# yanivw12/gs2mesh

Hardware: AMD Instinct MI355X
Metric: stereo-pair renders/sec + TSDF Mvoxel-updates/sec (higher is better)
Workload: dtype f32

## Files before the change

### gs2mesh_amd/csrc/tsdf_api.hip

```cpp
#include <math.h>
#include <stdio.h>
#include <string.h>

#include <mutex>
#include <vector>

#include "../../include/gs2mesh_amd.h"
#include "tsdf_common.h"
#include "tsdf_internal.h"
#include "roctx_ranges.h"

#define HIPCHK(expr)                                                                          \
    do {                                                                                      \
        hipError_t e__ = (expr);                                                              \
        if (e__ != hipSuccess) {                                                              \
            gs2m_set_error("%s failed: %s (%s:%d)", #expr, hipGetErrorString(e__), __FILE__, __LINE__); \
            return 1;                                                                         \
        }                                                                                     \
    } while (0)

struct gs2m_tsdf {
    int device = 0;
    double voxel_length = 0, sdf_trunc = 0, unit_length = 0;
    int color_type = 1, resolution = 16, stride = 4;
// ... 30 lines not shown

static hipEvent_t tsdf_ev_get(gs2m_tsdf* t) {
    if (!t->ev_free.empty()) {
        hipEvent_t e = t->ev_free.back();
        t->ev_free.pop_back();
        return e;
    }
    hipEvent_t e;
    if (hipEventCreate(&e) != hipSuccess) return nullptr;
    return e;
}

static bool invert4x4(const double* m, double* inv) {
    double a[16];
    a[0] = m[5] * m[10] * m[15] - m[5] * m[11] * m[14] - m[9] * m[6] * m[15] + m[9] * m[7] * m[14] + m[13] * m[6] * m[11] - m[13] * m[7] * m[10];
    a[4] = -m[4] * m[10] * m[15] + m[4] * m[11] * m[14] + m[8] * m[6] * m[15] - m[8] * m[7] * m[14] - m[12] * m[6] * m[11] + m[12] * m[7] * m[10];
    a[8] = m[4] * m[9] * m[15] - m[4] * m[11] * m[13] - m[8] * m[5] * m[15] + m[8] * m[7] * m[13] + m[12] * m[5] * m[11] - m[12] * m[7] * m[9];
    a[12] = -m[4] * m[9] * m[14] + m[4] * m[10] * m[13] + m[8] * m[5] * m[14] - m[8] * m[6] * m[13] - m[12] * m[5] * m[10] + m[12] * m[6] * m[9];
    a[1] = -m[1] * m[10] * m[15] + m[1] * m[11] * m[14] + m[9] * m[2] * m[15] - m[9] * m[3] * m[14] - m[13] * m[2] * m[11] + m[13] * m[3] * m[10];
    a[5] = m[0] * m[10] * m[15] - m[0] * m[11] * m[14] - m[8] * m[2] * m[15] + m[8] * m[3] * m[14] + m[12] * m[2] * m[11] - m[12] * m[3] * m[10];
    a[9] = -m[0] * m[9] * m[15] + m[0] * m[11] * m[13] + m[8] * m[1] * m[15] - m[8] * m[3] * m[13] - m[12] * m[1] * m[11] + m[12] * m[3] * m[9];
    a[13] = m[0] * m[9] * m[14] - m[0] * m[10] * m[13] - m[8] * m[1] * m[14] + m[8] * m[2] * m[13] + m[12] * m[1] * m[10] - m[12] * m[2] * m[9];
    a[2] = m[1] * m[6] * m[15] - m[1] * m[7] * m[14] - m[5] * m[2] * m[15] + m[5] * m[3] * m[14] + m[13] * m[2] * m[7] - m[13] * m[3] * m[6];
    a[6] = -m[0] * m[6] * m[15] + m[0] * m[7] * m[14] + m[4] * m[2] * m[15] - m[4] * m[3] * m[14] - m[12] * m[2] * m[7] + m[12] * m[3] * m[6];
    a[10] = m[0] * m[5] * m[15] - m[0] * m[7] * m[13] - m[4] * m[1] * m[15] + m[4] * m[3] * m[13] + m[12] * m[1] * m[7] - m[12] * m[3] * m[5];
    a[14] = -m[0] * m[5] * m[14] + m[0] * m[6] * m[13] + m[4] * m[1] * m[14] - m[4] * m[2] * m[13] - m[12] * m[1] * m[6] + m[12] * m[2] * m[5];
    a[3] = -m[1] * m[6] * m[11] + m[1] * m[7] * m[10] + m[5] * m[2] * m[11] - m[5] * m[3] * m[10] - m[9] * m[2] * m[7] + m[9] * m[3] * m[6];
    a[7] = m[0] * m[6] * m[11] - m[0] * m[7] * m[10] - m[4] * m[2] * m[11] + m[4] * m[3] * m[10] + m[8] * m[2] * m[7] - m[8] * m[3] * m[6];
    a[11] = -m[0] * m[5] * m[11] + m[0] * m[7] * m[9] + m[4] * m[1] * m[11] - m[4] * m[3] * m[9] - m[8] * m[1] * m[7] + m[8] * m[3] * m[5];
    a[15] = m[0] * m[5] * m[10] - m[0] * m[6] * m[9] - m[4] * m[1] * m[10] + m[4] * m[2] * m[9] + m[8] * m[1] * m[6] - m[8] * m[2] * m[5];
    double det = m[0] * a[0] + m[1] * a[4] + m[2] * a[8] + m[3] * a[12];
    if (det == 0) return false;
    det = 1.0 / det;
    for (int i = 0; i < 16; i++) inv[i] = a[i] * det;
    return true;
}

static int zero_state(gs2m_tsdf* t, hipStream_t st, bool whole_pool, long long keep_first = -1) {
    TsdfVolume& V = t->V;
    if (whole_pool) {
        HIPCHK(hipMemsetAsync(V.tsdf, 0, sizeof(float) * (size_t)V.max_blocks * GS2M_TSDF_VOX, st));
        HIPCHK(hipMemsetAsync(V.weight, 0, sizeof(float) * (size_t)V.max_blocks * GS2M_TSDF_VOX, st));
        if (V.rgb) HIPCHK(hipMemsetAsync(V.rgb, 0, sizeof(unsigned) * 3 * (size_t)V.max_blocks * GS2M_TSDF_VOX, st));
        HIPCHK(hipMemsetAsync(V.halo, 0, (size_t)V.max_blocks, st));
    } else if (keep_first < 0) {
        gs2m_launch_tsdf_clear_used(st, V);
    } else {
        gs2m_launch_tsdf_clear_from(st, V, (unsigned)keep_first);
    }
    HIPCHK(hipMemsetAsync(V.hash_keys, 0xff, sizeof(unsigned long long) * (size_t)V.hash_cap, st));
    HIPCHK(hipMemsetAsync(V.hash_vals, 0xff, sizeof(int) * (size_t)V.hash_cap, st));
    HIPCHK(hipMemsetAsync(V.stamp, 0, sizeof(unsigned) * (size_t)V.hash_cap, st));
    HIPCHK(hipMemsetAsync(V.fmask, 0, sizeof(unsigned long long) * (size_t)V.hash_cap, st));
    HIPCHK(hipMemsetAsync(V.counters, 0, sizeof(unsigned) * 4, st));
    HIPCHK(hipMemsetAsync(V.totals, 0, sizeof(unsigned long long), st));
    return 0;
}

extern "C" int gs2m_tsdf_create(gs2m_tsdf** out, double voxel_length, double sdf_trunc, int color_type,
                                int volume_unit_resolution, int depth_sampling_stride, int64_t max_blocks,
                                int device) {
    if (!out) {
        gs2m_set_error("gs2m_tsdf_create: out is NULL");
        return 1;
    }
    if (volume_unit_resolution != GS2M_TSDF_RES) {
        gs2m_set_error("volume_unit_resolution %d not supported (kernels are specialised for 16, Open3D's default)",
                       volume_unit_resolution);
        return 1;
    }
    if (!(voxel_length > 0) || !(sdf_trunc > 0) || depth_sampling_stride < 1 || max_blocks < 1 ||
        max_blocks > (1ll << 30) || (color_type != GS2M_TSDF_COLOR_NONE && color_type != GS2M_TSDF_COLOR_RGB8)) {
        gs2m_set_error("gs2m_tsdf_create: bad argument");
        return 1;
    }
    HIPCHK(hipSetDevice(device));
    gs2m_tsdf* t = new gs2m_tsdf();
    t->device = device;
    t->voxel_length = voxel_length;
    t->sdf_trunc = sdf_trunc;
    t->unit_length = voxel_length * volume_unit_resolution;
    t->color_type = color_type;
    t->stride = depth_sampling_stride;
    memset(&t->V, 0, sizeof(t->V));
    TsdfVolume& V = t->V;
    V.max_blocks = (unsigned)max_blocks;
    unsigned cap = 1024;
    while ((uint64_t)cap < 2ull * (uint64_t)max_blocks) cap <<= 1;
    V.hash_cap = cap;
    V.has_color = color_type == GS2M_TSDF_COLOR_RGB8;
    const size_t nvox = (size_t)max_blocks * GS2M_TSDF_VOX;
    bool ok = hipMalloc((void**)&V.tsdf, sizeof(float) * nvox) == hipSuccess &&
              hipMalloc((void**)&V.weight, sizeof(float) * nvox) == hipSuccess &&
              (!V.has_color || hipMalloc((void**)&V.rgb, sizeof(unsigned) * 3 * nvox) == hipSuccess) &&
              hipMalloc((void**)&V.block_keys, sizeof(int) * 3 * (size_t)max_blocks) == hipSuccess &&
              hipMalloc((void**)&V.halo, (size_t)max_blocks) == hipSuccess &&
              hipMalloc((void**)&V.hash_keys, sizeof(unsigned long long) * (size_t)cap) == hipSuccess &&
              hipMalloc((void**)&V.hash_vals, sizeof(int) * (size_t)cap) == hipSuccess &&
              hipMalloc((void**)&V.stamp, sizeof(unsigned) * (size_t)cap) == hipSuccess &&
              hipMalloc((void**)&V.touched, sizeof(unsigned) * (size_t)cap) == hipSuccess &&
              hipMalloc((void**)&V.fmask, sizeof(unsigned long long) * (size_t)cap) == hipSuccess &&
              hipMalloc((void**)&t->d_bframes, sizeof(TsdfBatchFrame) * GS2M_TSDF_MAX_BATCH) == hipSuccess &&
              hipHostMalloc((void**)&t->h_bframes, sizeof(TsdfBatchFrame) * GS2M_TSDF_MAX_BATCH * gs2m_tsdf::kRing) == hipSuccess &&
              hipMalloc((void**)&V.counters, sizeof(unsigned) * 4) == hipSuccess &&
              hipMalloc((void**)&V.totals, sizeof(unsigned long long)) == hipSuccess &&
              hipMalloc((void**)&t->d_mc, gs2m_mc_tables_bytes()) == hipSuccess &&
              hipMalloc((void**)&t->d_blk_tris, sizeof(unsigned) * (size_t)max_blocks) == hipSuccess &&
              hipMalloc((void**)&t->d_ntri, sizeof(unsigned long long)) == hipSuccess &&
              hipHostMalloc((void**)&t->h_counters, sizeof(unsigned) * 4) == hipSuccess &&
              hipHostMalloc((void**)&t->h_totals, sizeof(unsigned long long)) == hipSuccess;
    if (!ok) {
        gs2m_set_error("gs2m_tsdf_create: out of device memory for %lld blocks (%.1f MiB)", (long long)max_blocks,
                       (double)nvox * 20.0 / 1048576.0);
        gs2m_tsdf_destroy(t);
        return 1;
    }
    {
        std::vector<unsigned char> tab(gs2m_mc_tables_bytes());
        if (!gs2m_mc_tables_fill(tab.data()) ||
            hipMemcpy(t->d_mc, tab.data(), tab.size(), hipMemcpyHostToDevice) != hipSuccess) {
            gs2m_set_error("gs2m_tsdf_create: marching-cubes table generation failed");
            gs2m_tsdf_destroy(t);
            return 1;
        }
    }
    if (zero_state(t, (hipStream_t)0, true)) {
        gs2m_tsdf_destroy(t);
        return 1;
    }
    HIPCHK(hipStreamSynchronize((hipStream_t)0));
    *out = t;
    return 0;
}

extern "C" int gs2m_tsdf_destroy(gs2m_tsdf* t) {
    if (!t) return 0;
    TsdfVolume& V = t->V;
    (void)hipFree(V.tsdf);
    (void)hipFree(V.weight);
    (void)hipFree(V.rgb);
    (void)hipFree(V.block_keys);
    (void)hipFree(V.halo);
    (void)hipFree(V.hash_keys);
    (void)hipFree(V.hash_vals);
    (void)hipFree(V.stamp);
    (void)hipFree(V.touched);
    (void)hipFree(V.fmask);
    (void)hipFree(t->d_bframes);
    (void)hipHostFree(t->h_bframes);
    for (auto e : t->ring_done)
        if (e) (void)hipEventDestroy(e);
    (void)hipFree(V.counters);
    (void)hipFree(V.totals);
    (void)hipFree(t->d_mc);
    (void)hipFree(t->d_blk_tris);
    (void)hipFree(t->d_ntri);
    (void)hipFree(t->mesh_scratch);
// ... 111 lines not shown
    }
    {
        Gs2mRange rg("gs2m:tsdf_integrate");
        gs2m_launch_tsdf_integrate(st, t->n_cu * 7, t->V, f, depth, color, mask);
    }
    if (tm) {
        (void)hipEventRecord(e3, st);
        t->ev_live.push_back({0, e0, e1, 1});
        t->ev_live.push_back({1, e2, e3, 1});
    }
    return 0;
}

extern "C" int gs2m_tsdf_integrate_batch(gs2m_tsdf* t, int n_frames, const float* const* depth, const uint8_t* const* color,
                                         const uint8_t* const* mask, int width, int height, double fx, double fy, double cx,
                                         double cy, const double* extrinsics_w2c, double depth_scale, double depth_trunc,
                                         double min_depth, gs2m_stream stream) {
    if (!t || n_frames < 0 || (n_frames > 0 && (!depth || !extrinsics_w2c))) {
        gs2m_set_error("gs2m_tsdf_integrate_batch: NULL argument");
        return 1;
    }
    if (t->V.has_color && n_frames > 0 && !color) {
        gs2m_set_error("[ScalableTSDFVolume::Integrate] Unsupported image format.");
        return 1;
    }
    if (n_frames > 0 && (width <= 0 || height <= 0 || width > 65535 || height > 65535 || !(fx != 0) || !(fy != 0) || !(depth_scale != 0))) {
        gs2m_set_error("gs2m_tsdf_integrate_batch: bad intrinsics / size (the sweep packs pixel coordinates in 16 bits: <= 65535)");
        return 1;
    }
    HIPCHK(hipSetDevice(t->device));
    hipStream_t st = (hipStream_t)stream;
    for (int f0 = 0; f0 < n_frames; f0 += GS2M_TSDF_MAX_BATCH) {
        const int nf = n_frames - f0 < GS2M_TSDF_MAX_BATCH ? n_frames - f0 : GS2M_TSDF_MAX_BATCH;
        const unsigned slot = t->ring_next++ % gs2m_tsdf::kRing;
        if (t->ring_done[slot]) HIPCHK(hipEventSynchronize(t->ring_done[slot]));
        else HIPCHK(hipEventCreateWithFlags(&t->ring_done[slot], hipEventDisableTiming));
        TsdfBatchFrame* hb = t->h_bframes + (size_t)slot * GS2M_TSDF_MAX_BATCH;
        for (int k = 0; k < nf; ++k) {
            const int i = f0 + k;
            if (!depth[i] || (t->V.has_color && !color[i])) {
                gs2m_set_error("gs2m_tsdf_integrate_batch: frame %d has a NULL image", i);
                return 1;
            }
            const unsigned char* m = mask ? mask[i] : nullptr;
            if (fill_frame(t, hb[k].f, width, height, fx, fy, cx, cy, extrinsics_w2c + 16 * (size_t)i, depth_scale, depth_trunc,
                           min_depth, m != nullptr))
                return 1;
            hb[k].depth = depth[i];
            hb[k].color = color ? color[i] : nullptr;
            hb[k].mask = m;
        }
        HIPCHK(hipMemcpyAsync(t->d_bframes, hb, sizeof(TsdfBatchFrame) * nf, hipMemcpyHostToDevice, st));
        HIPCHK(hipEventRecord(t->ring_done[slot], st));
        HIPCHK(hipMemsetAsync(t->V.counters + 1, 0, sizeof(unsigned), st));
        HIPCHK(hipMemsetAsync(t->V.counters + 3, 0, sizeof(unsigned), st));
        hipEvent_t e0 = nullptr, e1 = nullptr, e2 = nullptr, e3 = nullptr;
        if (t->timing) {
            e0 = tsdf_ev_get(t);
            e1 = tsdf_ev_get(t);
            e2 = tsdf_ev_get(t);
            e3 = tsdf_ev_get(t);
        }
        const bool tm = e0 && e1 && e2 && e3;
        if (tm) (void)hipEventRecord(e0, st);
        {
            Gs2mRange rg("gs2m:tsdf_touch_batch");
            gs2m_launch_tsdf_touch_batch(st, t->V, hb[0].f, nf, t->d_bframes);
        }
        if (tm) {
            (void)hipEventRecord(e1, st);
            (void)hipEventRecord(e2, st);
        }
        {
            Gs2mRange rg("gs2m:tsdf_integrate_batch");
            gs2m_launch_tsdf_integrate_batch(st, t->n_cu, t->V, t->d_bframes);
        }
        if (tm) {
            (void)hipEventRecord(e3, st);
            t->ev_live.push_back({0, e0, e1, nf});
            t->ev_live.push_back({1, e2, e3, nf});
        }
    }
    return 0;
}

extern "C" int gs2m_tsdf_set_stage_timing(gs2m_tsdf* t, int enable) {
    if (!t) {
        gs2m_set_error("null handle");
        return 1;
    }
    t->timing = enable != 0;
    return 0;
}

extern "C" int gs2m_tsdf_stage_times(gs2m_tsdf* t, gs2m_stream stream, double* total_ms, int64_t* launches) {
    if (!t || !total_ms || !launches) {
        gs2m_set_error("gs2m_tsdf_stage_times: NULL argument");
        return 1;
    }
    HIPCHK(hipStreamSynchronize((hipStream_t)stream));
    for (auto& p : t->ev_live) {
        float ms = 0.f;
        if (hipEventElapsedTime(&ms, p.a, p.b) == hipSuccess && (p.stage == 0 || p.stage == 1)) {
            total_ms[p.stage] += ms;
            launches[p.stage] += p.frames;
        }
        t->ev_free.push_back(p.a);
        t->ev_free.push_back(p.b);
// ... 504 lines not shown
```

### gs2mesh_amd/csrc/tsdf_common.h

```cpp
#pragma once
#include "platform.h"

#define GS2M_TSDF_RES 16
#define GS2M_TSDF_VOX 4096
#define GS2M_TSDF_EMPTY 0xffffffffffffffffull
#define GS2M_TSDF_KEY_BIAS (1 << 20)

struct TsdfVolume {
    float* tsdf;
    float* weight;
    unsigned* rgb;
    int* block_keys;
    unsigned char* halo;
    unsigned long long* hash_keys;
    int* hash_vals;
    unsigned* stamp;
    unsigned* touched;
    unsigned long long* fmask;
    unsigned* counters;
    unsigned long long* totals;
    unsigned hash_cap;
    unsigned max_blocks;
    int has_color;
};

struct TsdfFrame {
    double pose[12];
    double fx, fy, cx, cy;
    double unit_length, sdf_trunc, depth_trunc;
    float E[12];
    float fx_f, fy_f, cx_f, cy_f, fx_inv_f, fy_inv_f;
    float voxel_length_f, half_voxel_length_f, sdf_trunc_f, sdf_trunc_inv_f;
    float Es02, Es12, Es22;
    float safe_w, safe_h;
    float depth_scale_f, min_depth_f;
    float depth_trunc_up_f;
    int W, H, stride, nx, ny;
    unsigned frame_id;
    int use_mask, use_min;
};

struct TsdfBatchFrame {
    TsdfFrame f;
    const float* depth;
    const unsigned char* color;
    const unsigned char* mask;
};
#define GS2M_TSDF_MAX_BATCH 64

#define GS2M_TSDF_VINDEX(x, y, z) (((((z) >> 2) * 16 + ((x) >> 2) * 4 + ((y) >> 2)) * 64) + ((z)&3) * 16 + ((x)&3) * 4 + ((y)&3))

GS2M_DEVICE unsigned long long tsdf_pack_key(int bx, int by, int bz) {
    return ((unsigned long long)(unsigned)(bx + GS2M_TSDF_KEY_BIAS) << 42) |
           ((unsigned long long)(unsigned)(by + GS2M_TSDF_KEY_BIAS) << 21) |
           (unsigned long long)(unsigned)(bz + GS2M_TSDF_KEY_BIAS);
}
GS2M_DEVICE bool tsdf_key_in_range(int bx, int by, int bz) {
    const int B = GS2M_TSDF_KEY_BIAS;
    return bx >= -B && bx < B && by >= -B && by < B && bz >= -B && bz < B;
}
GS2M_DEVICE unsigned tsdf_hash(unsigned long long k) {
    k ^= k >> 33;
    k *= 0xff51afd7ed558ccdull;
    k ^= k >> 33;
    k *= 0xc4ceb9fe1a85ec53ull;
    k ^= k >> 33;
    return (unsigned)k;
}
```

### gs2mesh_amd/csrc/tsdf_kernels.h

```cpp
#pragma once
#include "tsdf_common.h"

GS2M_DEVICE float tsdf_fetch_depth(const float* __restrict__ depth, const unsigned char* __restrict__ mask,
                                   const TsdfFrame& f, int u, int v) {
    const size_t p = (size_t)v * f.W + u;
    float d = depth[p];
    if (f.use_mask && mask[p] == 0) d = d * 0.0f;
    if (f.use_min && d < f.min_depth_f) d = 0.0f;
    if (f.depth_scale_f != 1.0f) d /= f.depth_scale_f;
    if (d >= f.depth_trunc_up_f) d = 0.0f;
    return d;
}

GS2M_DEVICE unsigned tsdf_find_or_insert(const TsdfVolume& V, unsigned long long key, int bx, int by, int bz) {
    const unsigned mask = V.hash_cap - 1u;
    unsigned h = tsdf_hash(key) & mask;
    for (unsigned probe = 0; probe < V.hash_cap; ++probe, h = (h + 1u) & mask) {
        unsigned long long k = V.hash_keys[h];
        if (k == key) return h;
        if (k == GS2M_TSDF_EMPTY) {
            const unsigned long long prev = atomicCAS(&V.hash_keys[h], GS2M_TSDF_EMPTY, key);
            if (prev == GS2M_TSDF_EMPTY) {
                const unsigned slot = atomicAdd(&V.counters[0], 1u);
                if (slot < V.max_blocks) {
// ... 103 lines not shown
        return;
    }
    const int ny = whi[1] - wlo[1] + 1, nz = whi[2] - wlo[2] + 1;
    const int nyz = ny * nz;
    const int total = (int)total_ll;
    for (int base = 0; base < total; base += 64) {
        const int c = base + lane;
        if (c >= total) continue;
        const int cx = c / nyz, rem = c - cx * nyz;
        const int cy = rem / nz;
        const int bx = wlo[0] + cx, by = wlo[1] + cy, bz = wlo[2] + (rem - cy * nz);
        int in_any = 0;
#pragma unroll 4
        for (int k = 0; k < n_keep; ++k)
            in_any |= (int)(bx >= stg->lo[0][k]) & (int)(bx <= stg->hi[0][k]) & (int)(by >= stg->lo[1][k]) &
                      (int)(by <= stg->hi[1][k]) & (int)(bz >= stg->lo[2][k]) & (int)(bz <= stg->hi[2][k]);
        const bool inside = in_any != 0;
        if (!inside) continue;
        if (!tsdf_key_in_range(bx, by, bz)) {
            atomicOr(&V.counters[2], 4u);
            continue;
        }
        const unsigned h = tsdf_find_or_insert(V, tsdf_pack_key(bx, by, bz), bx, by, bz);
        if (h == 0xffffffffu) continue;
        if (batch_bit < 0) {
            if (V.stamp[h] != f.frame_id) V.stamp[h] = f.frame_id;
        } else {
            const unsigned long long bit = 1ull << batch_bit;
            if (!(V.fmask[h] & bit)) atomicOr(&V.fmask[h], bit);
        }
    }
}

GS2M_KERNEL void __launch_bounds__(256)
k_tsdf_touch(TsdfVolume V, TsdfFrame f, const float* __restrict__ depth, const unsigned char* __restrict__ mask) {
    __shared__ TouchStage stage_all[4];
    tsdf_touch_body(V, f, depth, mask, stage_all, -1);
}

GS2M_KERNEL void __launch_bounds__(256)
k_tsdf_touch_batch(TsdfVolume V, const TsdfBatchFrame* __restrict__ frames) {
    __shared__ TouchStage stage_all[4];
    const TsdfBatchFrame& bf = frames[blockIdx.y];
    tsdf_touch_body(V, bf.f, bf.depth, bf.mask, stage_all, (int)blockIdx.y);
}


GS2M_KERNEL void __launch_bounds__(1024)
k_tsdf_compact(TsdfVolume V, unsigned frame_id) {
    __shared__ unsigned wave_cnt[16];
    __shared__ unsigned wg_base;
    const int tid = (int)threadIdx.x, lane = tid & 63, wave = tid >> 6;
    const unsigned h = blockIdx.x * 1024u + (unsigned)tid;
    const bool t = h < V.hash_cap && (frame_id ? V.stamp[h] == frame_id : V.fmask[h] != 0ull);
    const unsigned long long m = gs2m_ballot(t ? 1 : 0);
    if (lane == 0) wave_cnt[wave] = (unsigned)gs2m_popc64(m);
    __syncthreads();
    if (tid == 0) {
        unsigned s = 0;
        for (int k = 0; k < 16; ++k) {
            const unsigned c = wave_cnt[k];
            wave_cnt[k] = s;
            s += c;
        }
        wg_base = s ? atomicAdd(&V.counters[1], s) : 0u;
    }
    __syncthreads();
    if (t) {
        const unsigned rank = (unsigned)gs2m_popc64(m & ((1ull << lane) - 1ull));
        V.touched[wg_base + wave_cnt[wave] + rank] = h;
    }
}

GS2M_KERNEL void __launch_bounds__(256)
k_tsdf_integrate(TsdfVolume V, TsdfFrame f, const float* __restrict__ depth, const unsigned char* __restrict__ color,
                 const unsigned char* __restrict__ mask) {
    __shared__ float s_p0[16], s_p1[16];
    const int tid = (int)threadIdx.x;
    const int lane = tid & 63, wave = tid >> 6;
    const int lz = lane >> 4, lx = (lane >> 2) & 3, ly = lane & 3;
    const unsigned n_touched = V.counters[1];
    const int last_pix = f.W * f.H - 1;
    for (unsigned it = blockIdx.x; it < n_touched; it += gridDim.x) {
        const unsigned h = V.touched[it];
        const unsigned long long key = V.hash_keys[h];
        const int slot = V.hash_vals[h];
        if (slot < 0) continue;
        const int bx = (int)((key >> 42) & 0x1fffffull) - GS2M_TSDF_KEY_BIAS;
        const int by = (int)((key >> 21) & 0x1fffffull) - GS2M_TSDF_KEY_BIAS;
        const int bz = (int)(key & 0x1fffffull) - GS2M_TSDF_KEY_BIAS;
        const double ox = (double)bx * f.unit_length, oy = (double)by * f.unit_length, oz = (double)bz * f.unit_length;
        const float p2 = (float)(f.half_voxel_length_f + oz);
        __syncthreads();
        if (tid < 16) s_p0[tid] = (float)(f.half_voxel_length_f + f.voxel_length_f * tid + ox);
        else if (tid < 32) s_p1[tid - 16] = (float)(f.half_voxel_length_f + f.voxel_length_f * (tid - 16) + oy);
        __syncthreads();
        float* bt = V.tsdf + (size_t)slot * GS2M_TSDF_VOX;
        float* bw = V.weight + (size_t)slot * GS2M_TSDF_VOX;
        unsigned* bc = V.rgb + (size_t)slot * 3 * GS2M_TSDF_VOX;
#pragma unroll 1
        for (int g = 0; g < 4; ++g) {
            int pix[4], vi[4];
            float zc[4], mult[4], d[4], tnew[4];
            const int z0 = g * 4;
#pragma unroll
            for (int k = 0; k < 4; ++k) {
                const int mb = g * 16 + wave * 4 + k;
                const int x = wave * 4 + lx, y = k * 4 + ly;
                vi[k] = mb * 64 + lane;
                const float p0 = s_p0[x];
                const float p1 = s_p1[y];
                float pc0 = f.E[0] * p0 + f.E[1] * p1 + f.E[2] * p2 + f.E[3] * 1.f;
                float pc1 = f.E[4] * p0 + f.E[5] * p1 + f.E[6] * p2 + f.E[7] * 1.f;
                float pc2 = f.E[8] * p0 + f.E[9] * p1 + f.E[10] * p2 + f.E[11] * 1.f;
                for (int s = 0; s < z0; ++s) {
                    pc0 += f.Es02;
                    pc1 += f.Es12;
                    pc2 += f.Es22;
                }
#pragma unroll
                for (int s = 0; s < 3; ++s) {
                    if (s < lz) {
                        pc0 += f.Es02;
// ... 20 lines not shown
                d[k] = 0.0f;
                if (pix[k] >= 0) {
                    float dd = depth[pix[k]];
                    if (f.use_mask && mask[pix[k]] == 0) dd = dd * 0.0f;
                    if (f.use_min && dd < f.min_depth_f) dd = 0.0f;
                    if (f.depth_scale_f != 1.0f) dd /= f.depth_scale_f;
                    if (dd >= f.depth_trunc_up_f) dd = 0.0f;
                    d[k] = dd;
                }
            }
            bool upd[4];
#pragma unroll
            for (int k = 0; k < 4; ++k) {
                const float sdf = (d[k] - zc[k]) * mult[k];
                upd[k] = pix[k] >= 0 && d[k] > 0.0f && sdf > -f.sdf_trunc_f;
                tnew[k] = fminf(1.0f, sdf * f.sdf_trunc_inv_f);
            }
            float w[4], t[4];
            unsigned c0[4], c1[4], c2[4], rgbp[4];
#pragma unroll
            for (int k = 0; k < 4; ++k) {
                if (upd[k]) {
                    w[k] = bw[vi[k]];
                    t[k] = bt[vi[k]];
                    if (V.has_color) {
                        c0[k] = bc[vi[k]];
                        c1[k] = bc[GS2M_TSDF_VOX + vi[k]];
                        c2[k] = bc[2 * GS2M_TSDF_VOX + vi[k]];
                        const unsigned char* c = color + 3 * (size_t)pix[k];
                        rgbp[k] = pix[k] < last_pix ? gs2m_load_u32_unaligned(c)
                                                    : ((unsigned)c[0] | ((unsigned)c[1] << 8) | ((unsigned)c[2] << 16));
                    }
                }
            }
#pragma unroll
            for (int k = 0; k < 4; ++k) {
                if (upd[k]) {
                    bt[vi[k]] = (t[k] * w[k] + tnew[k]) / (w[k] + 1.0f);
                    if (V.has_color) {
                        bc[vi[k]] = c0[k] + (rgbp[k] & 0xffu);
                        bc[GS2M_TSDF_VOX + vi[k]] = c1[k] + ((rgbp[k] >> 8) & 0xffu);
                        bc[2 * GS2M_TSDF_VOX + vi[k]] = c2[k] + ((rgbp[k] >> 16) & 0xffu);
                    }
                    bw[vi[k]] = w[k] + 1.0f;
                }
            }
        }
    }
    if (blockIdx.x == 0 && tid == 0) V.totals[0] += n_touched;
}

GS2M_KERNEL void __launch_bounds__(256)
k_tsdf_integrate_batch(TsdfVolume V, const TsdfBatchFrame* __restrict__ frames) {
    __shared__ float s_p0[16], s_p1[16];
    const int tid = (int)threadIdx.x;
    const int x = (tid >> 4) & 15, y = tid & 15;
    __shared__ unsigned s_it;
    const unsigned n_touched = V.counters[1] * 4u;
    const TsdfFrame& f0 = frames[0].f;
    for (;;) {
        __syncthreads();
        if (tid == 0) s_it = atomicAdd(&V.counters[3], 1u);
        __syncthreads();
        const unsigned it = s_it;
        if (it >= n_touched) break;
        const int zq = (int)(it & 3u);
        const unsigned h = V.touched[it >> 2];
        const unsigned long long key = V.hash_keys[h];
        const int slot = V.hash_vals[h];
        const unsigned long long fm = V.fmask[h];
        if (slot < 0) continue;
        const int bx = (int)((key >> 42) & 0x1fffffull) - GS2M_TSDF_KEY_BIAS;
        const int by = (int)((key >> 21) & 0x1fffffull) - GS2M_TSDF_KEY_BIAS;
        const int bz = (int)(key & 0x1fffffull) - GS2M_TSDF_KEY_BIAS;
        const double ox = (double)bx * f0.unit_length, oy = (double)by * f0.unit_length, oz = (double)bz * f0.unit_length;
        const float p2 = (float)(f0.half_voxel_length_f + oz);
        if (tid < 16) s_p0[tid] = (float)(f0.half_voxel_length_f + f0.voxel_length_f * tid + ox);
        else if (tid < 32) s_p1[tid - 16] = (float)(f0.half_voxel_length_f + f0.voxel_length_f * (tid - 16) + oy);
        __syncthreads();
        const float p0 = s_p0[x], p1 = s_p1[y];
        float* bt = V.tsdf + (size_t)slot * GS2M_TSDF_VOX;
        float* bw = V.weight + (size_t)slot * GS2M_TSDF_VOX;
        unsigned* bc = V.rgb + (size_t)slot * 3 * GS2M_TSDF_VOX;
        const int vi0 = GS2M_TSDF_VINDEX(x, y, 4 * zq);
        float w[4], t[4];
        unsigned c0[4], c1[4], c2[4];
#pragma unroll
        for (int j = 0; j < 4; ++j) {
            w[j] = bw[vi0 + 16 * j];
            t[j] = bt[vi0 + 16 * j];
            c0[j] = c1[j] = c2[j] = 0u;
            if (V.has_color) {
                c0[j] = bc[vi0 + 16 * j];
                c1[j] = bc[GS2M_TSDF_VOX + vi0 + 16 * j];
                c2[j] = bc[2 * GS2M_TSDF_VOX + vi0 + 16 * j];
            }
        }
        struct Probe {
            int fi;
            int pix[4];
            unsigned uv[4];
            float zc[4], d[4];
        };
        auto probe = [&](const int fi, Probe& P) __attribute__((always_inline)) {
            const TsdfBatchFrame& bf = frames[fi];
            const TsdfFrame& f = bf.f;
            const float* __restrict__ depth = bf.depth;
            const unsigned char* __restrict__ mask = bf.mask;
            P.fi = fi;
            float pc0 = f.E[0] * p0 + f.E[1] * p1 + f.E[2] * p2 + f.E[3] * 1.f;
            float pc1 = f.E[4] * p0 + f.E[5] * p1 + f.E[6] * p2 + f.E[7] * 1.f;
            float pc2 = f.E[8] * p0 + f.E[9] * p1 + f.E[10] * p2 + f.E[11] * 1.f;
            for (int s = 0; s < 4 * zq; ++s) {
                pc0 += f.Es02;
                pc1 += f.Es12;
                pc2 += f.Es22;
            }
#pragma unroll
            for (int j = 0; j < 4; ++j) {
                P.pix[j] = -1;
                P.uv[j] = 0u;
                P.zc[j] = pc2;
                if (!(pc2 <= 0)) {
                    const float u_f = pc0 * f.fx_f / pc2 + f.cx_f + 0.5f;
                    const float v_f = pc1 * f.fy_f / pc2 + f.cy_f + 0.5f;
                    if (u_f >= 0.0001f && u_f < f.safe_w && v_f >= 0.0001f && v_f < f.safe_h) {
                        const int uu = (int)u_f, vv = (int)v_f;
                        P.uv[j] = (unsigned)uu | ((unsigned)vv << 16);
                        P.pix[j] = vv * f.W + uu;
                    }
                }
                pc0 += f.Es02;
                pc1 += f.Es12;
                pc2 += f.Es22;
            }
#pragma unroll
            for (int j = 0; j < 4; ++j) {
                P.d[j] = 0.0f;
                if (P.pix[j] >= 0) {
                    float dd = depth[P.pix[j]];
                    if (f.use_mask && mask[P.pix[j]] == 0) dd = dd * 0.0f;
                    P.d[j] = dd;
                }
            }
        };
        auto apply = [&](Probe& P) __attribute__((always_inline)) {
            const TsdfBatchFrame& bf = frames[P.fi];
            const TsdfFrame& f = bf.f;
            const unsigned char* __restrict__ color = bf.color;
            const int last_pix = f.W * f.H - 1;
            unsigned rgbp[4];
            bool upd[4];
            float tnew[4];
#pragma unroll
            for (int j = 0; j < 4; ++j) {
                upd[j] = false;
                tnew[j] = 0.0f;
                rgbp[j] = 0u;
                float dd = P.d[j];
                if (P.pix[j] >= 0) {
                    if (f.use_min && dd < f.min_depth_f) dd = 0.0f;
                    if (f.depth_scale_f != 1.0f) dd /= f.depth_scale_f;
                    if (dd >= f.depth_trunc_up_f) dd = 0.0f;
                }
                if (P.pix[j] >= 0 && dd > 0.0f) {
                    const float xx = ((int)(P.uv[j] & 0xffffu) - f.cx_f) * f.fx_inv_f;
                    const float yy = ((int)(P.uv[j] >> 16) - f.cy_f) * f.fy_inv_f;
                    const float mult = sqrtf(xx * xx + yy * yy + 1.0f);
                    const float sdf = (dd - P.zc[j]) * mult;
                    if (sdf > -f.sdf_trunc_f) {
                        upd[j] = true;
                        tnew[j] = fminf(1.0f, sdf * f.sdf_trunc_inv_f);
                        if (V.has_color) {
                            const unsigned char* c = color + 3 * (size_t)P.pix[j];
                            rgbp[j] = P.pix[j] < last_pix ? gs2m_load_u32_unaligned(c)
                                                          : ((unsigned)c[0] | ((unsigned)c[1] << 8) | ((unsigned)c[2] << 16));
                        }
                    }
                }
            }
#pragma unroll
            for (int j = 0; j < 4; ++j) {
                if (upd[j]) {
                    t[j] = (t[j] * w[j] + tnew[j]) / (w[j] + 1.0f);
                    c0[j] += rgbp[j] & 0xffu;
                    c1[j] += (rgbp[j] >> 8) & 0xffu;
                    c2[j] += (rgbp[j] >> 16) & 0xffu;
                    w[j] = w[j] + 1.0f;
                }
            }
        };
        unsigned long long todo = fm;
        Probe A, B;
        if (todo != 0ull) {
            probe(__ffsll(todo) - 1, A);
            todo &= todo - 1ull;
            while (todo != 0ull) {
                probe(__ffsll(todo) - 1, B);
                todo &= todo - 1ull;
                apply(A);
                if (todo == 0ull) {
                    A = B;
                    break;
                }
                probe(__ffsll(todo) - 1, A);
                todo &= todo - 1ull;
                apply(B);
                if (todo == 0ull) break;
            }
            apply(A);
        }
#pragma unroll
        for (int j = 0; j < 4; ++j) {
            bw[vi0 + 16 * j] = w[j];
            bt[vi0 + 16 * j] = t[j];
            if (V.has_color) {
                bc[vi0 + 16 * j] = c0[j];
                bc[GS2M_TSDF_VOX + vi0 + 16 * j] = c1[j];
                bc[2 * GS2M_TSDF_VOX + vi0 + 16 * j] = c2[j];
            }
        }
        if (tid == 0 && zq == 0) atomicAdd(&V.totals[0], (unsigned long long)gs2m_popc64(fm));
    }
}

GS2M_KERNEL void __launch_bounds__(256)
k_tsdf_clear_fmask(TsdfVolume V) {
    const unsigned n = V.counters[1];
    for (unsigned i = blockIdx.x * 256u + threadIdx.x; i < n; i += gridDim.x * 256u) V.fmask[V.touched[i]] = 0ull;
}

GS2M_KERNEL void __launch_bounds__(256)
k_tsdf_clear_used(TsdfVolume V) {
    unsigned n = V.counters[0];
    if (n > V.max_blocks) n = V.max_blocks;
    const float4 z = {0.f, 0.f, 0.f, 0.f};
    for (unsigned slot = blockIdx.x; slot < n; slot += gridDim.x) {
        float4* t4 = reinterpret_cast<float4*>(V.tsdf + (size_t)slot * GS2M_TSDF_VOX);
        float4* w4 = reinterpret_cast<float4*>(V.weight + (size_t)slot * GS2M_TSDF_VOX);
        for (int i = (int)threadIdx.x; i < GS2M_TSDF_VOX / 4; i += 256) {
            t4[i] = z;
            w4[i] = z;
        }
        if (V.has_color) {
            float4* c4 = reinterpret_cast<float4*>(V.rgb + (size_t)slot * 3 * GS2M_TSDF_VOX);
            for (int i = (int)threadIdx.x; i < 3 * GS2M_TSDF_VOX / 4; i += 256) c4[i] = z;
        }
        if (threadIdx.x == 0) V.halo[slot] = 0;
    }
}

GS2M_KERNEL void __launch_bounds__(256)
k_tsdf_clear_from(TsdfVolume V, unsigned first) {
    unsigned n = V.counters[0];
    if (n > V.max_blocks) n = V.max_blocks;
    const float4 z = {0.f, 0.f, 0.f, 0.f};
    for (unsigned slot = first + blockIdx.x; slot < n; slot += gridDim.x) {
        float4* t4 = reinterpret_cast<float4*>(V.tsdf + (size_t)slot * GS2M_TSDF_VOX);
        float4* w4 = reinterpret_cast<float4*>(V.weight + (size_t)slot * GS2M_TSDF_VOX);
        for (int i = (int)threadIdx.x; i < GS2M_TSDF_VOX / 4; i += 256) {
            t4[i] = z;
            w4[i] = z;
        }
        if (V.has_color) {
            float4* c4 = reinterpret_cast<float4*>(V.rgb + (size_t)slot * 3 * GS2M_TSDF_VOX);
            for (int i = (int)threadIdx.x; i < 3 * GS2M_TSDF_VOX / 4; i += 256) c4[i] = z;
        }
        if (threadIdx.x == 0) V.halo[slot] = 0;
    }
}

GS2M_KERNEL void __launch_bounds__(256)
k_tsdf_clear_gap(TsdfVolume V, unsigned upto) {
    unsigned first = V.counters[0];
    if (upto > V.max_blocks) upto = V.max_blocks;
    const float4 z = {0.f, 0.f, 0.f, 0.f};
    for (unsigned slot = first + blockIdx.x; slot < upto; slot += gridDim.x) {
        float4* t4 = reinterpret_cast<float4*>(V.tsdf + (size_t)slot * GS2M_TSDF_VOX);
        float4* w4 = reinterpret_cast<float4*>(V.weight + (size_t)slot * GS2M_TSDF_VOX);
        for (int i = (int)threadIdx.x; i < GS2M_TSDF_VOX / 4; i += 256) {
            t4[i] = z;
            w4[i] = z;
// ... 185 lines not shown
```

### gs2mesh_amd/csrc/tsdf_kernels.hip

```cpp
#include "tsdf_kernels.h"
#include "tsdf_extract.h"
#include "mesh_kernels.h"
#include "tsdf_internal.h"
#include <math.h>

void gs2m_launch_tsdf_touch(hipStream_t st, const TsdfVolume& V, const TsdfFrame& f, const float* depth,
                            const unsigned char* mask) {
    const int n = f.nx * f.ny;
    GS2M_LAUNCH(k_tsdf_touch, dim3((n + 255) / 256), dim3(256), 0, st, V, f, depth, mask);
    GS2M_LAUNCH(k_tsdf_compact, dim3((V.hash_cap + 1023u) / 1024u), dim3(1024), 0, st, V, f.frame_id);
}
void gs2m_launch_tsdf_integrate(hipStream_t st, int n_wg, const TsdfVolume& V, const TsdfFrame& f,
                                const float* depth, const unsigned char* color, const unsigned char* mask) {
    GS2M_LAUNCH(k_tsdf_integrate, dim3(n_wg), dim3(256), 0, st, V, f, depth, color, mask);
}
void gs2m_launch_tsdf_touch_batch(hipStream_t st, const TsdfVolume& V, const TsdfFrame& f, int n_frames,
                                  const TsdfBatchFrame* frames) {
    const int n = f.nx * f.ny;
    GS2M_LAUNCH(k_tsdf_touch_batch, dim3((n + 255) / 256, n_frames), dim3(256), 0, st, V, frames);
    GS2M_LAUNCH(k_tsdf_compact, dim3((V.hash_cap + 1023u) / 1024u), dim3(1024), 0, st, V, 0u);
}
void gs2m_launch_tsdf_integrate_batch(hipStream_t st, int n_cu, const TsdfVolume& V, const TsdfBatchFrame* frames) {
    GS2M_LAUNCH(k_tsdf_integrate_batch, dim3(n_cu * 6), dim3(256), 0, st, V, frames);
    GS2M_LAUNCH(k_tsdf_clear_fmask, dim3(16), dim3(256), 0, st, V);
}
void gs2m_launch_tsdf_clear_used(hipStream_t st, const TsdfVolume& V) {
    GS2M_LAUNCH(k_tsdf_clear_used, dim3(2048), dim3(256), 0, st, V);
}
void gs2m_launch_tsdf_pack(hipStream_t st, unsigned n, const TsdfVolume& V, const int* keys, int form, float* buf, long long* ibuf) {
    if (form == GS2M_XF_SUM_PACKED) GS2M_LAUNCH(k_tsdf_pack<GS2M_XF_SUM_PACKED>, dim3(n), dim3(256), 0, st, V, keys, buf, ibuf);
    else if (form == GS2M_XF_RAW_F32) GS2M_LAUNCH(k_tsdf_pack<GS2M_XF_RAW_F32>, dim3(n), dim3(256), 0, st, V, keys, buf, ibuf);
    else GS2M_LAUNCH(k_tsdf_pack<GS2M_XF_SUM_F32>, dim3(n), dim3(256), 0, st, V, keys, buf, ibuf);
}
void gs2m_launch_tsdf_unpack(hipStream_t st, unsigned n, const TsdfVolume& V, const int* keys, int form, const float* buf,
                             const long long* ibuf, int halo) {
    if (form == GS2M_XF_SUM_PACKED) GS2M_LAUNCH(k_tsdf_unpack<GS2M_XF_SUM_PACKED>, dim3(n), dim3(256), 0, st, V, keys, buf, ibuf, halo);
    else if (form == GS2M_XF_RAW_F32) GS2M_LAUNCH(k_tsdf_unpack<GS2M_XF_RAW_F32>, dim3(n), dim3(256), 0, st, V, keys, buf, ibuf, halo);
    else GS2M_LAUNCH(k_tsdf_unpack<GS2M_XF_SUM_F32>, dim3(n), dim3(256), 0, st, V, keys, buf, ibuf, halo);
}
void gs2m_launch_tsdf_clear_from(hipStream_t st, const TsdfVolume& V, unsigned first) {
    GS2M_LAUNCH(k_tsdf_clear_from, dim3(1024), dim3(256), 0, st, V, first);
}
void gs2m_launch_tsdf_clear_gap(hipStream_t st, const TsdfVolume& V, unsigned upto) {
    GS2M_LAUNCH(k_tsdf_clear_gap, dim3(256), dim3(256), 0, st, V, upto);
}
void gs2m_launch_tsdf_owned_keys(hipStream_t st, unsigned n, const TsdfVolume& V, int* keys) {
    GS2M_LAUNCH(k_tsdf_owned_keys, dim3((n + 255u) / 256u), dim3(256), 0, st, V, n, keys);
}

void gs2m_launch_tsdf_block_map(hipStream_t st, const TsdfVolume& V, const int* lo, const int* dim, unsigned char* cells, unsigned n_cells,
                                unsigned flags, unsigned win_hash, int rank, unsigned frames_local, unsigned frames_base) {
    const unsigned wg = (V.max_blocks + 255u) / 256u;
    GS2M_LAUNCH(k_tsdf_block_map, dim3(wg < 256u ? (wg ? wg : 1u) : 256u), dim3(256), 0, st, V, lo[0], lo[1], lo[2], dim[0], dim[1], dim[2], cells,
                n_cells, flags, win_hash, rank, frames_local, frames_base);
}
void gs2m_launch_tsdf_map_keys(hipStream_t st, const int* lo, const int* dim, unsigned char* cells, unsigned n_cells, int* keys, unsigned max_keys) {
    GS2M_LAUNCH(k_tsdf_map_keys, dim3(1), dim3(1024), 0, st, lo[0], lo[1], lo[2], dim[1], dim[2], cells, n_cells, keys, max_keys);
}

size_t gs2m_mc_tables_bytes() { return sizeof(McDevTables); }
bool gs2m_mc_tables_fill(void* host_buf) {
    McTables T;
    if (!mc_generate(&T)) return false;
    McDevTables* D = (McDevTables*)host_buf;
    memcpy(D->tri, T.tri, sizeof(T.tri));
    memcpy(D->ntri, T.ntri, sizeof(T.ntri));
    return true;
}
void gs2m_launch_mc_count(hipStream_t st, const TsdfVolume& V, const McDevTables* T, unsigned n_blocks,
                          unsigned* blk_tris, unsigned long long* n_total) {
    GS2M_LAUNCH(k_mc_count, dim3(n_blocks), dim3(256), 0, st, V, T, n_blocks, blk_tris);
    GS2M_LAUNCH(k_mc_scan, dim3(1), dim3(1024), 0, st, blk_tris, n_blocks, n_total);
}
// ... 59 lines not shown
```

Baseline: 4119.

## Sort touched blocks heavy-first and prefetch work-queue index in batch integrate

Batched compaction now runs in two passes. The first counts touched blocks per frame-count class, the second writes them to the touched list in descending order of how many frames see each block, so the dynamic work queue hands out expensive blocks first and reduces tail imbalance. The integrate kernel fetches the next work item while processing the current one using double-buffered shared slots, computes voxel coordinates in registers instead of through shared memory with a different thread-to-voxel mapping, and defers colour accumulation by one frame. Counter resets move from host memsets into the fmask-clear kernel. In exchange there is an extra full hash-table pass and a larger counters array.

```diff
diff --git a/gs2mesh_amd/csrc/tsdf_api.hip b/gs2mesh_amd/csrc/tsdf_api.hip
--- a/gs2mesh_amd/csrc/tsdf_api.hip
+++ b/gs2mesh_amd/csrc/tsdf_api.hip
@@ -106,7 +106,7 @@
     HIPCHK(hipMemsetAsync(V.hash_vals, 0xff, sizeof(int) * (size_t)V.hash_cap, st));
     HIPCHK(hipMemsetAsync(V.stamp, 0, sizeof(unsigned) * (size_t)V.hash_cap, st));
     HIPCHK(hipMemsetAsync(V.fmask, 0, sizeof(unsigned long long) * (size_t)V.hash_cap, st));
-    HIPCHK(hipMemsetAsync(V.counters, 0, sizeof(unsigned) * 4, st));
+    HIPCHK(hipMemsetAsync(V.counters, 0, sizeof(unsigned) * GS2M_TSDF_NCOUNTERS, st));
     HIPCHK(hipMemsetAsync(V.totals, 0, sizeof(unsigned long long), st));
     return 0;
 }
@@ -156,7 +156,7 @@
               hipMalloc((void**)&V.fmask, sizeof(unsigned long long) * (size_t)cap) == hipSuccess &&
               hipMalloc((void**)&t->d_bframes, sizeof(TsdfBatchFrame) * GS2M_TSDF_MAX_BATCH) == hipSuccess &&
               hipHostMalloc((void**)&t->h_bframes, sizeof(TsdfBatchFrame) * GS2M_TSDF_MAX_BATCH * gs2m_tsdf::kRing) == hipSuccess &&
-              hipMalloc((void**)&V.counters, sizeof(unsigned) * 4) == hipSuccess &&
+              hipMalloc((void**)&V.counters, sizeof(unsigned) * GS2M_TSDF_NCOUNTERS) == hipSuccess &&
               hipMalloc((void**)&V.totals, sizeof(unsigned long long)) == hipSuccess &&
               hipMalloc((void**)&t->d_mc, gs2m_mc_tables_bytes()) == hipSuccess &&
               hipMalloc((void**)&t->d_blk_tris, sizeof(unsigned) * (size_t)max_blocks) == hipSuccess &&
@@ -374,8 +374,6 @@
         }
         HIPCHK(hipMemcpyAsync(t->d_bframes, hb, sizeof(TsdfBatchFrame) * nf, hipMemcpyHostToDevice, st));
         HIPCHK(hipEventRecord(t->ring_done[slot], st));
-        HIPCHK(hipMemsetAsync(t->V.counters + 1, 0, sizeof(unsigned), st));
-        HIPCHK(hipMemsetAsync(t->V.counters + 3, 0, sizeof(unsigned), st));
         hipEvent_t e0 = nullptr, e1 = nullptr, e2 = nullptr, e3 = nullptr;
         if (t->timing) {
             e0 = tsdf_ev_get(t);
diff --git a/gs2mesh_amd/csrc/tsdf_common.h b/gs2mesh_amd/csrc/tsdf_common.h
--- a/gs2mesh_amd/csrc/tsdf_common.h
+++ b/gs2mesh_amd/csrc/tsdf_common.h
@@ -47,6 +47,10 @@
     const unsigned char* mask;
 };
 #define GS2M_TSDF_MAX_BATCH 64
+#define GS2M_TSDF_NCLS (GS2M_TSDF_MAX_BATCH + 1)
+#define GS2M_TSDF_CNT_CLASS 4
+#define GS2M_TSDF_CNT_CURSOR (GS2M_TSDF_CNT_CLASS + GS2M_TSDF_NCLS)
+#define GS2M_TSDF_NCOUNTERS (GS2M_TSDF_CNT_CURSOR + GS2M_TSDF_NCLS)
 
 #define GS2M_TSDF_VINDEX(x, y, z) (((((z) >> 2) * 16 + ((x) >> 2) * 4 + ((y) >> 2)) * 64) + ((z)&3) * 16 + ((x)&3) * 4 + ((y)&3))
 
diff --git a/gs2mesh_amd/csrc/tsdf_kernels.h b/gs2mesh_amd/csrc/tsdf_kernels.h
--- a/gs2mesh_amd/csrc/tsdf_kernels.h
+++ b/gs2mesh_amd/csrc/tsdf_kernels.h
@@ -179,7 +179,7 @@
     __shared__ unsigned wg_base;
     const int tid = (int)threadIdx.x, lane = tid & 63, wave = tid >> 6;
     const unsigned h = blockIdx.x * 1024u + (unsigned)tid;
-    const bool t = h < V.hash_cap && (frame_id ? V.stamp[h] == frame_id : V.fmask[h] != 0ull);
+    const bool t = h < V.hash_cap && V.stamp[h] == frame_id;
     const unsigned long long m = gs2m_ballot(t ? 1 : 0);
     if (lane == 0) wave_cnt[wave] = (unsigned)gs2m_popc64(m);
     __syncthreads();
@@ -196,6 +196,47 @@
     if (t) {
         const unsigned rank = (unsigned)gs2m_popc64(m & ((1ull << lane) - 1ull));
         V.touched[wg_base + wave_cnt[wave] + rank] = h;
+    }
+}
+
+GS2M_KERNEL void __launch_bounds__(1024)
+k_tsdf_class_count(TsdfVolume V) {
+    __shared__ unsigned cls[GS2M_TSDF_NCLS];
+    const int tid = (int)threadIdx.x;
+    if (tid < GS2M_TSDF_NCLS) cls[tid] = 0u;
+    __syncthreads();
+    const unsigned h = blockIdx.x * 1024u + (unsigned)tid;
+    const unsigned long long fm = h < V.hash_cap ? V.fmask[h] : 0ull;
+    if (fm != 0ull) atomicAdd(&cls[gs2m_popc64(fm)], 1u);
+    __syncthreads();
+    if (tid < GS2M_TSDF_NCLS && cls[tid]) atomicAdd(&V.counters[GS2M_TSDF_CNT_CLASS + tid], cls[tid]);
+}
+
+GS2M_KERNEL void __launch_bounds__(1024)
+k_tsdf_compact_heavy_first(TsdfVolume V) {
+    __shared__ unsigned cls[GS2M_TSDF_NCLS], total[GS2M_TSDF_NCLS], base[GS2M_TSDF_NCLS];
+    const int tid = (int)threadIdx.x;
+    if (tid < GS2M_TSDF_NCLS) {
+        cls[tid] = 0u;
+        total[tid] = V.counters[GS2M_TSDF_CNT_CLASS + tid];
+    }
+    __syncthreads();
+    const unsigned h = blockIdx.x * 1024u + (unsigned)tid;
+    const unsigned long long fm = h < V.hash_cap ? V.fmask[h] : 0ull;
+    const int c = gs2m_popc64(fm);
+    const unsigned rank = fm != 0ull ? atomicAdd(&cls[c], 1u) : 0u;
+    __syncthreads();
+    if (tid < GS2M_TSDF_NCLS) {
+        unsigned start = 0u;
+        for (int k = tid + 1; k < GS2M_TSDF_NCLS; ++k) start += total[k];
+        const unsigned n = cls[tid];
+        base[tid] = start + (n ? atomicAdd(&V.counters[GS2M_TSDF_CNT_CURSOR + tid], n) : 0u);
+        if (tid == 0 && blockIdx.x == 0) V.counters[1] = start;
+    }
+    __syncthreads();
+    if (fm != 0ull) {
+        const unsigned at = base[c] + rank;
+        if (at < V.hash_cap) V.touched[at] = h;
     }
 }
 
@@ -322,33 +363,39 @@
 
 GS2M_KERNEL void __launch_bounds__(256)
 k_tsdf_integrate_batch(TsdfVolume V, const TsdfBatchFrame* __restrict__ frames) {
-    __shared__ float s_p0[16], s_p1[16];
     const int tid = (int)threadIdx.x;
-    const int x = (tid >> 4) & 15, y = tid & 15;
-    __shared__ unsigned s_it;
+    const int x = 8 * (tid >> 7) + ((tid >> 3) & 4) + ((tid >> 2) & 3), y = 8 * ((tid >> 6) & 1) + ((tid >> 2) & 4) + (tid & 3);
     const unsigned n_touched = V.counters[1] * 4u;
     const TsdfFrame& f0 = frames[0].f;
-    for (;;) {
+    __shared__ unsigned s_it[2];
+    if (tid == 0) s_it[0] = atomicAdd(&V.counters[3], 1u);
+    __syncthreads();
+    unsigned it = (unsigned)gs2m_uniform((int)s_it[0]), par = 1u;
+    auto advance = [&](const unsigned next_it) __attribute__((always_inline)) {
+        if (tid == 0) s_it[par] = next_it;
         __syncthreads();
-        if (tid == 0) s_it = atomicAdd(&V.counters[3], 1u);
-        __syncthreads();
-        const unsigned it = s_it;
-        if (it >= n_touched) break;
+        it = (unsigned)gs2m_uniform((int)s_it[par]);
+        par ^= 1u;
+    };
+    while (it < n_touched) {
+        unsigned next_it = 0u;
+        if (tid == 0) next_it = atomicAdd(&V.counters[3], 1u);
         const int zq = (int)(it & 3u);
         const unsigned h = V.touched[it >> 2];
         const unsigned long long key = V.hash_keys[h];
         const int slot = V.hash_vals[h];
         const unsigned long long fm = V.fmask[h];
-        if (slot < 0) continue;
+        if (slot < 0) {
+            advance(next_it);
+            continue;
+        }
         const int bx = (int)((key >> 42) & 0x1fffffull) - GS2M_TSDF_KEY_BIAS;
         const int by = (int)((key >> 21) & 0x1fffffull) - GS2M_TSDF_KEY_BIAS;
         const int bz = (int)(key & 0x1fffffull) - GS2M_TSDF_KEY_BIAS;
         const double ox = (double)bx * f0.unit_length, oy = (double)by * f0.unit_length, oz = (double)bz * f0.unit_length;
         const float p2 = (float)(f0.half_voxel_length_f + oz);
-        if (tid < 16) s_p0[tid] = (float)(f0.half_voxel_length_f + f0.voxel_length_f * tid + ox);
-        else if (tid < 32) s_p1[tid - 16] = (float)(f0.half_voxel_length_f + f0.voxel_length_f * (tid - 16) + oy);
-        __syncthreads();
-        const float p0 = s_p0[x], p1 = s_p1[y];
+        const float p0 = (float)(f0.half_voxel_length_f + f0.voxel_length_f * x + ox);
+        const float p1 = (float)(f0.half_voxel_length_f + f0.voxel_length_f * y + oy);
         float* bt = V.tsdf + (size_t)slot * GS2M_TSDF_VOX;
         float* bw = V.weight + (size_t)slot * GS2M_TSDF_VOX;
         unsigned* bc = V.rgb + (size_t)slot * 3 * GS2M_TSDF_VOX;
@@ -372,6 +419,7 @@
             unsigned uv[4];
             float zc[4], d[4];
         };
+        unsigned pend[4] = {0u, 0u, 0u, 0u};
         auto probe = [&](const int fi, Probe& P) __attribute__((always_inline)) {
             const TsdfBatchFrame& bf = frames[fi];
             const TsdfFrame& f = bf.f;
@@ -451,11 +499,12 @@
             }
 #pragma unroll
             for (int j = 0; j < 4; ++j) {
+                c0[j] += pend[j] & 0xffu;
+                c1[j] += (pend[j] >> 8) & 0xffu;
+                c2[j] += (pend[j] >> 16) & 0xffu;
+                pend[j] = rgbp[j];
                 if (upd[j]) {
                     t[j] = (t[j] * w[j] + tnew[j]) / (w[j] + 1.0f);
-                    c0[j] += rgbp[j] & 0xffu;
-                    c1[j] += (rgbp[j] >> 8) & 0xffu;
-                    c2[j] += (rgbp[j] >> 16) & 0xffu;
                     w[j] = w[j] + 1.0f;
                 }
             }
@@ -485,12 +534,13 @@
             bw[vi0 + 16 * j] = w[j];
             bt[vi0 + 16 * j] = t[j];
             if (V.has_color) {
-                bc[vi0 + 16 * j] = c0[j];
-                bc[GS2M_TSDF_VOX + vi0 + 16 * j] = c1[j];
-                bc[2 * GS2M_TSDF_VOX + vi0 + 16 * j] = c2[j];
+                bc[vi0 + 16 * j] = c0[j] + (pend[j] & 0xffu);
+                bc[GS2M_TSDF_VOX + vi0 + 16 * j] = c1[j] + ((pend[j] >> 8) & 0xffu);
+                bc[2 * GS2M_TSDF_VOX + vi0 + 16 * j] = c2[j] + ((pend[j] >> 16) & 0xffu);
             }
         }
         if (tid == 0 && zq == 0) atomicAdd(&V.totals[0], (unsigned long long)gs2m_popc64(fm));
+        advance(next_it);
     }
 }
 
@@ -498,6 +548,8 @@
 k_tsdf_clear_fmask(TsdfVolume V) {
     const unsigned n = V.counters[1];
     for (unsigned i = blockIdx.x * 256u + threadIdx.x; i < n; i += gridDim.x * 256u) V.fmask[V.touched[i]] = 0ull;
+    if (blockIdx.x == 0)
+        for (unsigned i = 3u + threadIdx.x; i < GS2M_TSDF_NCOUNTERS; i += 256u) V.counters[i] = 0u;
 }
 
 GS2M_KERNEL void __launch_bounds__(256)
diff --git a/gs2mesh_amd/csrc/tsdf_kernels.hip b/gs2mesh_amd/csrc/tsdf_kernels.hip
--- a/gs2mesh_amd/csrc/tsdf_kernels.hip
+++ b/gs2mesh_amd/csrc/tsdf_kernels.hip
@@ -18,7 +18,8 @@
                                   const TsdfBatchFrame* frames) {
     const int n = f.nx * f.ny;
     GS2M_LAUNCH(k_tsdf_touch_batch, dim3((n + 255) / 256, n_frames), dim3(256), 0, st, V, frames);
-    GS2M_LAUNCH(k_tsdf_compact, dim3((V.hash_cap + 1023u) / 1024u), dim3(1024), 0, st, V, 0u);
+    GS2M_LAUNCH(k_tsdf_class_count, dim3((V.hash_cap + 1023u) / 1024u), dim3(1024), 0, st, V);
+    GS2M_LAUNCH(k_tsdf_compact_heavy_first, dim3((V.hash_cap + 1023u) / 1024u), dim3(1024), 0, st, V);
 }
 void gs2m_launch_tsdf_integrate_batch(hipStream_t st, int n_cu, const TsdfVolume& V, const TsdfBatchFrame* frames) {
     GS2M_LAUNCH(k_tsdf_integrate_batch, dim3(n_cu * 6), dim3(256), 0, st, V, frames);
```

Result: no change. 4157, median of 6 (+0.9%).
